# Ryan-Yanlong/DREAM-GNN

Hardware: AMD Instinct MI355X
Metric: GCMC+FGCN SpMM edges/sec and achieved HBM GB/s at 1/2/4/8 MI355X (higher is better)
Workload: dtype f32

## Files before the change

### dream_gnn_amd/csrc/dgmi_api.hip

```cpp
#include <hip/hip_runtime.h>
#include <limits.h>
#include <stdlib.h>
#include <string.h>

#include "dgmi.h"
#include "dgmi_bf16.h"
#include "dgmi_keep.h"
#include "dgmi_kernels.h"
#include "dgmi_tuning.h"

namespace {

inline hipStream_t as_stream(dgmi_stream_t s) { return static_cast<hipStream_t>(s); }

inline int from_hip(hipError_t e) { return e == hipSuccess ? DGMI_OK : DGMI_ERR_LAUNCH; }

long long env_ll(const char* name, long long dflt) {
  const char* e = getenv(name);
  return e != nullptr && e[0] != '\0' ? atoll(e) : dflt;
}

}

namespace dgmi {

Tuning& tuning() {
  static Tuning t = [] {
    Tuning v;
    v.sliced_rows = (int)env_ll("DGMI_SLICED_ROWS", 0);
    v.sliced_touch_lead = (int)env_ll("DGMI_SLICED_PF", -1);
    v.sliced_lpr = (int)env_ll("DGMI_SLICED_LPR", 0);
    v.sliced_no_off32 = getenv("DGMI_NO_OFF32") != nullptr ? 1 : 0;
    v.sliced_chunk_rows = env_ll("DGMI_SLICED_CHUNK_ROWS", 0);
    v.sliced_taper_rows = env_ll("DGMI_SLICED_TAPER_ROWS", 0);
    v.select_window_min = env_ll("DGMI_SELECT_WINDOW_MIN", 0);
    v.select_narrow_window = env_ll("DGMI_SELECT_NARROW_WINDOW", 0) != 0 ? 1 : 0;
    v.sort_plain_tiles = env_ll("DGMI_SORT_PLAIN_TILES", 0) != 0 ? 1 : 0;
    v.knn_screen_first = env_ll("DGMI_KNN_SCREEN_V1", 0) != 0 ? 1 : 0;
    v.knn_pool_chunks = env_ll("DGMI_KNN_POOL_CHUNKS", 0);
    return v;
  }();
  return t;
}

}

extern "C" {

DGMI_API int dgmi_set_tuning(const char* name, int64_t value) {
  if (name == nullptr) return DGMI_ERR_INVALID_ARG;
  dgmi::Tuning& t = dgmi::tuning();
  if (strcmp(name, "sliced_rows") == 0) t.sliced_rows = (int)value;
  else if (strcmp(name, "sliced_touch_lead") == 0) t.sliced_touch_lead = (int)value;
  else if (strcmp(name, "sliced_lpr") == 0) t.sliced_lpr = (int)value;
  else if (strcmp(name, "sliced_no_off32") == 0) t.sliced_no_off32 = value != 0;
  else if (strcmp(name, "sliced_chunk_rows") == 0) t.sliced_chunk_rows = value;
  else if (strcmp(name, "sliced_taper_rows") == 0) t.sliced_taper_rows = value;
  else if (strcmp(name, "select_window_min") == 0) t.select_window_min = value;
  else if (strcmp(name, "select_narrow_window") == 0) t.select_narrow_window = value != 0;
  else if (strcmp(name, "sort_plain_tiles") == 0) t.sort_plain_tiles = value != 0;
  else if (strcmp(name, "knn_screen_first") == 0) t.knn_screen_first = value != 0;
  else if (strcmp(name, "knn_pool_chunks") == 0) t.knn_pool_chunks = value;
  else return DGMI_ERR_INVALID_ARG;
  return DGMI_OK;
}

DGMI_API int dgmi_abi_version(void) { return DGMI_ABI_VERSION; }

DGMI_API const char* dgmi_status_string(int status) {
  switch (status) {
    case DGMI_OK: return "ok";
    case DGMI_ERR_INVALID_ARG: return "invalid argument (null pointer, negative size or ld < F)";
    case DGMI_ERR_TOO_LARGE: return "size does not fit the int32 id space";
    case DGMI_ERR_WORKSPACE: return "workspace missing or too small";
    case DGMI_ERR_LAUNCH: return "HIP launch failed";
    case DGMI_ERR_NO_DEVICE: return "no gfx950 device visible";
    default: return "unknown dgmi status";
  }
}

DGMI_API int dgmi_device_ok(void) {
  int n = 0;
  if (hipGetDeviceCount(&n) != hipSuccess || n <= 0) return 0;
  int dev = 0;
  if (hipGetDevice(&dev) != hipSuccess) return 0;
  hipDeviceProp_t prop;
  if (hipGetDeviceProperties(&prop, dev) != hipSuccess) return 0;
  return strncmp(prop.gcnArchName, "gfx950", 6) == 0 ? 1 : 0;
}

DGMI_API int dgmi_csr_from_coo_i32(const int32_t* row, const int32_t* col, int64_t E, int64_t n_rows,
                          int64_t n_cols, int32_t* indptr, int32_t* indices, int32_t* eid, void* workspace,
                          size_t* workspace_bytes, dgmi_stream_t stream) {
  if (E < 0 || n_rows < 0 || workspace_bytes == nullptr) return DGMI_ERR_INVALID_ARG;
  if (E > INT32_MAX || n_rows >= INT32_MAX || n_cols >= INT32_MAX) return DGMI_ERR_TOO_LARGE;
  if (workspace != nullptr) {
    if (indptr == nullptr) return DGMI_ERR_INVALID_ARG;
    if (E > 0 && (row == nullptr || col == nullptr || indices == nullptr || eid == nullptr))
      return DGMI_ERR_INVALID_ARG;
  }
  size_t need = 0;
  hipError_t err = dgmi::csr_from_coo_i32(row, col, E, n_rows, n_cols, indptr, indices, eid, nullptr,
                                          &need, as_stream(stream));
  if (err != hipSuccess) return DGMI_ERR_LAUNCH;
  if (workspace == nullptr) {
    *workspace_bytes = need;
    return DGMI_OK;
  }
  if (*workspace_bytes < need) return DGMI_ERR_WORKSPACE;
  return from_hip(dgmi::csr_from_coo_i32(row, col, E, n_rows, n_cols, indptr, indices, eid, workspace,
                                         workspace_bytes, as_stream(stream)));
}

static bool epilogue_ok(int32_t act, const float* out_mask, int64_t ld_mask, int64_t F) {
  return (act == 0 || act == 1) && (out_mask == nullptr || ld_mask >= F);
}

static bool keep_args_ok(const int32_t* eid, const uint32_t* keep, int32_t n_keep) {
  if (n_keep < 0 || n_keep > dgmi::kMaxKeepSegs) return false;
  return n_keep == 0 || (eid != nullptr && keep != nullptr);
}

DGMI_API int dgmi_spmm_csr_f32(const int32_t* indptr, const int32_t* indices, const float* vals,
                      const int32_t* eid, const uint32_t* keep, int32_t n_keep,
                      const float* X, int64_t ldx, const float* src_scale,
                      const float* dst_scale, float* Y, int64_t ldy, int64_t n_dst,
                      int64_t n_src, int64_t F, int32_t act, float act_slope, const float* out_mask,
                      int64_t ld_mask, float out_mask_scale, dgmi_stream_t stream) {
  if (n_dst < 0 || n_src < 0 || F < 0 || !keep_args_ok(eid, keep, n_keep) || !epilogue_ok(act, out_mask, ld_mask, F))
    return DGMI_ERR_INVALID_ARG;
  if (n_dst >= INT32_MAX || n_src >= INT32_MAX || F > INT32_MAX) return DGMI_ERR_TOO_LARGE;
  if (n_dst == 0 || F == 0) return DGMI_OK;
  if (indptr == nullptr || Y == nullptr) return DGMI_ERR_INVALID_ARG;
  if (ldx < F || ldy < F) return DGMI_ERR_INVALID_ARG;
  if (X == nullptr && n_src > 0) return DGMI_ERR_INVALID_ARG;
  if (static_cast<const void*>(X) == static_cast<const void*>(Y)) return DGMI_ERR_INVALID_ARG;
  dgmi::SpmmArgs a{indptr, indices, vals, X, ldx, src_scale, dst_scale, Y, ldy, n_dst, n_src, F,
                   nullptr, 0, 0, nullptr, 0, eid, keep, n_keep, {act, act_slope, out_mask, ld_mask, out_mask_scale}};
  return from_hip(dgmi::spmm_csr_f32(a, as_stream(stream)));
}

DGMI_API int32_t dgmi_spmm_default_chunk(int64_t n_rows, int64_t nnz) {
  (void)n_rows;
  int64_t c = (nnz / 4096 + 63) / 64 * 64;
  if (c < 64) c = 64;
  if (c > 512) c = 512;
  return (int32_t)c;
}

static bool chunk_ok(int32_t chunk) { return chunk >= 16 && chunk <= 65536; }

DGMI_API size_t dgmi_spmm_plan_bytes(int64_t n_rows, int64_t nnz, int32_t chunk) {
  if (n_rows < 0 || nnz < 0 || !chunk_ok(chunk)) return 0;
  return dgmi::plan_bytes(n_rows, nnz, chunk);
}

DGMI_API size_t dgmi_spmm_partials_bytes(int64_t nnz, int32_t chunk, int64_t F) {
  if (nnz < 0 || F < 0 || !chunk_ok(chunk)) return 0;
  const size_t ldp = (size_t)((F + 3) / 4 * 4);
  const size_t b = (size_t)dgmi::plan_slots_cap(nnz, chunk) * ldp * sizeof(float);
  return b < 16 ? 16 : b;
}

DGMI_API int dgmi_spmm_plan_build(const int32_t* indptr, int64_t n_rows, int64_t nnz, int32_t chunk,
                                  void* plan, size_t plan_bytes, void* workspace,
                                  size_t* workspace_bytes, dgmi_stream_t stream) {
  if (n_rows < 0 || nnz < 0 || !chunk_ok(chunk) || workspace_bytes == nullptr)
    return DGMI_ERR_INVALID_ARG;
  if (n_rows >= INT32_MAX || nnz > INT32_MAX) return DGMI_ERR_TOO_LARGE;
  size_t need = 0;
  if (dgmi::spmm_plan_build(indptr, n_rows, nnz, chunk, nullptr, nullptr, &need, as_stream(stream)) !=
      hipSuccess)
    return DGMI_ERR_LAUNCH;
  if (workspace == nullptr) {
    *workspace_bytes = need;
    return DGMI_OK;
  }
  if (plan == nullptr || (indptr == nullptr && n_rows > 0)) return DGMI_ERR_INVALID_ARG;
  if (*workspace_bytes < need || plan_bytes < dgmi::plan_bytes(n_rows, nnz, chunk))
    return DGMI_ERR_WORKSPACE;
  return from_hip(dgmi::spmm_plan_build(indptr, n_rows, nnz, chunk, static_cast<int32_t*>(plan),
                                        workspace, workspace_bytes, as_stream(stream)));
}

DGMI_API int dgmi_spmm_csr_planned_f32(const int32_t* indptr, const int32_t* indices,
                                       const float* vals, const int32_t* eid, const uint32_t* keep,
                                       int32_t n_keep, const float* X, int64_t ldx,
                                       const float* src_scale, const float* dst_scale, float* Y,
                                       int64_t ldy, int64_t n_dst, int64_t n_src, int64_t F,
                                       int64_t nnz, int32_t chunk, const void* plan, void* partials,
                                       size_t partials_bytes, int32_t act, float act_slope,
                                       const float* out_mask, int64_t ld_mask, float out_mask_scale,
                                       dgmi_stream_t stream) {
  if (n_dst < 0 || n_src < 0 || F < 0 || nnz < 0 || !chunk_ok(chunk) || !keep_args_ok(eid, keep, n_keep) ||
      !epilogue_ok(act, out_mask, ld_mask, F))
    return DGMI_ERR_INVALID_ARG;
  if (n_dst >= INT32_MAX || n_src >= INT32_MAX || F > INT32_MAX || nnz > INT32_MAX)
    return DGMI_ERR_TOO_LARGE;
  if (n_dst == 0 || F == 0) return DGMI_OK;
  if (indptr == nullptr || Y == nullptr || plan == nullptr || partials == nullptr)
    return DGMI_ERR_INVALID_ARG;
  if (ldx < F || ldy < F) return DGMI_ERR_INVALID_ARG;
  if (X == nullptr && n_src > 0) return DGMI_ERR_INVALID_ARG;
  if (static_cast<const void*>(X) == static_cast<const void*>(Y)) return DGMI_ERR_INVALID_ARG;
  if (partials_bytes < dgmi_spmm_partials_bytes(nnz, chunk, F)) return DGMI_ERR_WORKSPACE;
  dgmi::SpmmArgs a{indptr, indices, vals, X, ldx, src_scale, dst_scale, Y, ldy, n_dst, n_src, F,
                   static_cast<const int32_t*>(plan), nnz, chunk, static_cast<float*>(partials),
                   (F + 3) / 4 * 4, eid, keep, n_keep, {act, act_slope, out_mask, ld_mask, out_mask_scale}};
  return from_hip(dgmi::spmm_csr_f32(a, as_stream(stream)));
}

static int64_t slice_width_for(int64_t n_cols, int32_t n_slices) {
  const int64_t w = (n_cols + n_slices - 1) / n_slices;
  return w > 0 ? w : 1;
}

DGMI_API int dgmi_csr_sliced_from_coo_i32(const int32_t* row, const int32_t* col, int64_t E, int64_t n_rows,
                                          int64_t n_cols, int32_t n_slices, int32_t* segptr,
                                          int32_t* indices, int32_t* eid, void* workspace,
                                          size_t* workspace_bytes, dgmi_stream_t stream) {
  if (E < 0 || n_rows < 0 || n_cols < 0 || n_slices < 1 || n_slices > 64 || workspace_bytes == nullptr)
    return DGMI_ERR_INVALID_ARG;
  if (E > INT32_MAX || n_cols >= INT32_MAX || n_rows * (int64_t)n_slices >= INT32_MAX) return DGMI_ERR_TOO_LARGE;
  if (workspace != nullptr) {
    if (segptr == nullptr) return DGMI_ERR_INVALID_ARG;
    if (E > 0 && (row == nullptr || col == nullptr || indices == nullptr || eid == nullptr))
      return DGMI_ERR_INVALID_ARG;
  }
  const int64_t width = slice_width_for(n_cols, n_slices);
  size_t need = 0;
  if (dgmi::csr_sliced_from_coo_i32(row, col, E, n_rows, n_cols, n_slices, width, segptr, indices, eid, nullptr,
                                    &need, as_stream(stream)) != hipSuccess)
    return DGMI_ERR_LAUNCH;
  if (workspace == nullptr) {
    *workspace_bytes = need;
    return DGMI_OK;
  }
  if (*workspace_bytes < need) return DGMI_ERR_WORKSPACE;
  return from_hip(dgmi::csr_sliced_from_coo_i32(row, col, E, n_rows, n_cols, n_slices, width, segptr, indices,
                                                eid, workspace, workspace_bytes, as_stream(stream)));
}

DGMI_API int dgmi_csr_sliced_from_csr_i32(const int32_t* indptr, const int32_t* indices, const int32_t* eid, int64_t E,
                                          int64_t n_rows, int64_t n_cols, int32_t n_slices, int32_t* segptr,
                                          int32_t* s_indices, int32_t* s_eid, void* workspace, size_t* workspace_bytes,
                                          dgmi_stream_t stream) {
  if (E < 0 || n_rows < 0 || n_cols < 0 || n_slices < 1 || n_slices > 64 || workspace_bytes == nullptr)
    return DGMI_ERR_INVALID_ARG;
  if (E > INT32_MAX || n_cols >= INT32_MAX || n_rows * (int64_t)n_slices >= INT32_MAX) return DGMI_ERR_TOO_LARGE;
  if (workspace != nullptr) {
    if (segptr == nullptr) return DGMI_ERR_INVALID_ARG;
    if (E > 0 && (indptr == nullptr || indices == nullptr || eid == nullptr || s_indices == nullptr || s_eid == nullptr))
      return DGMI_ERR_INVALID_ARG;
  }
  const int64_t width = slice_width_for(n_cols, n_slices);
  size_t need = 0;
  if (dgmi::csr_sliced_from_csr_i32(indptr, indices, eid, E, n_rows, n_cols, n_slices, width, segptr, s_indices, s_eid,
                                    nullptr, &need, as_stream(stream)) != hipSuccess)
    return DGMI_ERR_LAUNCH;
  if (workspace == nullptr) {
    *workspace_bytes = need;
    return DGMI_OK;
  }
  if (*workspace_bytes < need) return DGMI_ERR_WORKSPACE;
  return from_hip(dgmi::csr_sliced_from_csr_i32(indptr, indices, eid, E, n_rows, n_cols, n_slices, width, segptr, s_indices,
                                                s_eid, workspace, workspace_bytes, as_stream(stream)));
}

static int64_t sliced_chunk_rows(int64_t n_dst, int32_t n_slices, int64_t F) {
  const int64_t row_bytes = (int64_t)n_slices * ((F + 3) / 4 * 4) * (int64_t)sizeof(float);
  int64_t rows = ((int64_t)4096 << 20) / (row_bytes > 0 ? row_bytes : 1);
  rows = rows / 1024 * 1024;
  if (rows < 1024) rows = 1024;
  if (dgmi::tuning().sliced_chunk_rows > 0) rows = dgmi::tuning().sliced_chunk_rows;
  return rows < n_dst ? rows : n_dst;
}

DGMI_API size_t dgmi_spmm_sliced_planes_bytes(int64_t n_dst, int32_t n_slices, int64_t F) {
  if (n_dst < 0 || n_slices < 1 || F < 0) return 0;
  const size_t b = (size_t)sliced_chunk_rows(n_dst, n_slices, F) * (size_t)n_slices *
                   (size_t)((F + 3) / 4 * 4) * sizeof(float);
  return b < 16 ? 16 : b;
}

static int spmm_sliced(const int32_t* segptr, const int32_t* indices, const float* vals, const int32_t* eid, const uint32_t* keep,
                       int32_t n_keep, const void* X, int x_bytes, int64_t ldx, const float* src_scale, const float* dst_scale,
                       float* Y, int64_t ldy, int64_t n_dst, int64_t n_src, int64_t F, int32_t n_slices, int32_t column_passes,
                       int32_t id_multiplicity, void* planes, size_t planes_bytes, int32_t act, float act_slope,
                       const float* out_mask, int64_t ld_mask, float out_mask_scale, dgmi_stream_t stream) {
  const int cols = 16 / x_bytes;
  if (n_dst < 0 || n_src < 0 || F < 0 || n_slices < 1 || n_slices > 64 || !keep_args_ok(eid, keep, n_keep) ||
      !epilogue_ok(act, out_mask, ld_mask, F) || column_passes < 0 || column_passes > 1 || id_multiplicity < 0 ||
      id_multiplicity > 1)
    return DGMI_ERR_INVALID_ARG;
  if (id_multiplicity == 1 && (vals != nullptr || n_src > (int64_t)dgmi::kMultIdMask + 1)) return DGMI_ERR_INVALID_ARG;
  if (out_mask != nullptr && (ld_mask % 4 != 0 || (reinterpret_cast<uintptr_t>(out_mask) & 15))) return DGMI_ERR_INVALID_ARG;
  if (n_dst >= INT32_MAX || n_src >= INT32_MAX || F > INT32_MAX) return DGMI_ERR_TOO_LARGE;
  if (n_dst == 0 || F == 0) return DGMI_OK;
  if (segptr == nullptr || Y == nullptr || planes == nullptr) return DGMI_ERR_INVALID_ARG;
  if (X == nullptr && n_src > 0) return DGMI_ERR_INVALID_ARG;
  if (ldx < F || ldy < F || F % cols != 0 || ldx % cols != 0 || ldy % 4 != 0) return DGMI_ERR_INVALID_ARG;
  if ((reinterpret_cast<uintptr_t>(X) & 15) || (reinterpret_cast<uintptr_t>(Y) & 15) ||
      (reinterpret_cast<uintptr_t>(planes) & 15))
    return DGMI_ERR_INVALID_ARG;
  if (X == static_cast<const void*>(Y)) return DGMI_ERR_INVALID_ARG;
  if (planes_bytes < dgmi_spmm_sliced_planes_bytes(n_dst, n_slices, F)) return DGMI_ERR_WORKSPACE;
  dgmi::SlicedArgs a{segptr, indices, vals, X, x_bytes, ldx, src_scale, dst_scale, Y, ldy, n_dst, n_src, F, n_slices,
                     static_cast<float*>(planes), F, sliced_chunk_rows(n_dst, n_slices, F), eid, keep, n_keep,
                     {act, act_slope, out_mask, ld_mask, out_mask_scale}, column_passes == 1, id_multiplicity == 1};
  return from_hip(x_bytes == 4 ? dgmi::spmm_sliced_f32(a, as_stream(stream)) : dgmi::spmm_sliced_bf16(a, as_stream(stream)));
}

DGMI_API int dgmi_spmm_sliced_f32(const int32_t* segptr, const int32_t* indices, const float* vals,
                                  const int32_t* eid, const uint32_t* keep, int32_t n_keep,
                                  const float* X, int64_t ldx, const float* src_scale,
                                  const float* dst_scale, float* Y, int64_t ldy, int64_t n_dst,
                                  int64_t n_src, int64_t F, int32_t n_slices, int32_t column_passes,
                                  int32_t id_multiplicity, void* planes,
                                  size_t planes_bytes, int32_t act, float act_slope, const float* out_mask,
                                  int64_t ld_mask, float out_mask_scale, dgmi_stream_t stream) {
  return spmm_sliced(segptr, indices, vals, eid, keep, n_keep, X, 4, ldx, src_scale, dst_scale, Y, ldy, n_dst, n_src, F,
                     n_slices, column_passes, id_multiplicity, planes, planes_bytes, act, act_slope, out_mask, ld_mask,
                     out_mask_scale, stream);
}

DGMI_API int dgmi_rows_to_bf16(const float* X, int64_t ldx, const float* scale, int64_t n, int64_t F, uint16_t* out, int64_t ldo,
                               dgmi_stream_t stream) {
  if (n < 0 || F < 0 || F % 8 != 0 || ldx < F || ldo < F || ldx % 4 != 0 || ldo % 8 != 0) return DGMI_ERR_INVALID_ARG;
  if (F > INT32_MAX) return DGMI_ERR_TOO_LARGE;
  if (n == 0 || F == 0) return DGMI_OK;
  if (X == nullptr || out == nullptr) return DGMI_ERR_INVALID_ARG;
  if ((reinterpret_cast<uintptr_t>(X) & 15) || (reinterpret_cast<uintptr_t>(out) & 15)) return DGMI_ERR_INVALID_ARG;
  if (static_cast<const void*>(X) == static_cast<const void*>(out)) return DGMI_ERR_INVALID_ARG;
  return from_hip(dgmi::rows_to_bf16(X, ldx, scale, n, F, out, ldo, as_stream(stream)));
}

DGMI_API int dgmi_spmm_sliced_bf16(const int32_t* segptr, const int32_t* indices, const float* vals, const int32_t* eid,
                                   const uint32_t* keep, int32_t n_keep, const uint16_t* X, int64_t ldx,
                                   const float* dst_scale, float* Y, int64_t ldy, int64_t n_dst, int64_t n_src, int64_t F,
                                   int32_t n_slices, int32_t column_passes, int32_t id_multiplicity, void* planes,
                                   size_t planes_bytes, int32_t act, float act_slope, const float* out_mask,
                                   int64_t ld_mask, float out_mask_scale, dgmi_stream_t stream) {
  return spmm_sliced(segptr, indices, vals, eid, keep, n_keep, X, 2, ldx, nullptr, dst_scale, Y, ldy, n_dst, n_src, F,
                     n_slices, column_passes, id_multiplicity, planes, planes_bytes, act, act_slope, out_mask, ld_mask,
                     out_mask_scale, stream);
}

DGMI_API int dgmi_gather_concat_f32(const int32_t* src, const int32_t* dst, int64_t E, const float* A,
                                    int64_t lda, int64_t Fa, const float* B, int64_t ldb, int64_t Fb,
                                    float* out, int64_t ldo, dgmi_stream_t stream) {
  if (E < 0 || Fa < 0 || Fb < 0) return DGMI_ERR_INVALID_ARG;
  if (E > INT32_MAX || Fa + Fb > INT32_MAX) return DGMI_ERR_TOO_LARGE;
  if (E == 0 || Fa + Fb == 0) return DGMI_OK;
  if (src == nullptr || dst == nullptr || out == nullptr) return DGMI_ERR_INVALID_ARG;
  if ((Fa > 0 && A == nullptr) || (Fb > 0 && B == nullptr)) return DGMI_ERR_INVALID_ARG;
  if (lda < Fa || ldb < Fb || ldo < Fa + Fb) return DGMI_ERR_INVALID_ARG;
  return from_hip(dgmi::gather_concat_f32(src, dst, E, A, lda, Fa, B, ldb, Fb, out, ldo, as_stream(stream)));
}

DGMI_API int dgmi_gather_add_f32(const int32_t* src, const int32_t* dst, int64_t E, const float* A,
// ... 177 lines not shown
```

### dream_gnn_amd/csrc/dgmi_sliced.hip

```cpp
#include <hip/hip_runtime.h>
#include <stdint.h>

#include "dgmi_sliced_common.h"

namespace dgmi {
namespace {

template <bool OFF32>
__device__ __forceinline__ float4 ld_row(const float* __restrict__ X, const float* __restrict__ Xc, int idx, int64_t ldx,
                                         uint32_t row_bytes, uint32_t col_bytes) {
  if (OFF32) return *reinterpret_cast<const float4*>(reinterpret_cast<const char*>(X) + ((uint32_t)idx * row_bytes + col_bytes));
  return ld4(Xc + (int64_t)idx * ldx);
}

template <int LPR, int VALS, bool HAS_SS, bool KEEP, bool OFF32>
__global__ __launch_bounds__(kWave* kWavesPerBlock) void spmm_sliced_vec4_kernel(
    const int32_t* __restrict__ segptr, const int32_t* __restrict__ indices,
    const float* __restrict__ vals, const float* __restrict__ X, int64_t ldx,
    const float* __restrict__ src_scale, float* __restrict__ planes, int64_t ldp, int64_t n_dst,
    int64_t row_begin, int64_t row_end, int F, int n_slices, const int32_t* __restrict__ eid,
    const KeepSeg* __restrict__ keep, int n_keep, int touch_lead, SlicedRuns runs, int touch_group) {
  constexpr int G = kWave / LPR;
  constexpr bool HAS_VALS = VALS == 1;
  constexpr bool MULT = VALS == 2;
  constexpr bool WEIGHTED = HAS_VALS || HAS_SS || MULT;
  constexpr bool W_LANE = HAS_VALS || HAS_SS;
  constexpr int kIdMask = MULT ? (int)kMultIdMask : 0x7fffffff;
  const int lane = threadIdx.x & (kWave - 1);
  const int wave = threadIdx.x >> 6;
  const int grp = lane / LPR, glane = lane % LPR, gbase = grp * LPR;
  const int slice = (int)(blockIdx.x % (unsigned)n_slices);
  int64_t block = blockIdx.x / (unsigned)n_slices;
  if (touch_group > 0 &&
      touch_ahead<HAS_VALS, KEEP>(segptr, indices, vals, eid, n_dst, row_begin, row_end, slice, runs, touch_lead, touch_group,
                                  lane, wave, block))
    return;
  const SlicedRun run = sliced_run(runs, block, wave * G + grp);
  const int nr = run.rows;
  if (nr == 0) return;
  const int64_t row0 = row_begin + run.first;
  int col = ((int)blockIdx.y * LPR + glane) * 4;
  const bool col_ok = col < F;
  if (!col_ok) col = 0;
  const float* Xc = X + col;
  const uint32_t row_bytes = (uint32_t)ldx * 4u, col_bytes = (uint32_t)col * 4u;
  const int32_t* sp = segptr + (int64_t)slice * n_dst + row0;
  float* prow = planes + ((int64_t)slice * (row_end - row_begin) + (row0 - row_begin)) * ldp + col;

  const KeepPre first = first_seg<KEEP>(keep, n_keep);
  const int my_b = sp[glane < nr ? glane : nr];
  const int e_begin = __shfl(my_b, gbase, kWave);
  const int e_end = __shfl(my_b, gbase + nr, kWave);
  int r = 0;
  int next_b = __shfl(my_b, gbase + 1, kWave);
  float4 acc = make_float4(0.f, 0.f, 0.f, 0.f);
  int nxt_idx = 0;
  float nxt_w = 0.f;
  int last_row = -1;
  if (e_begin < e_end) {
    const int q = e_begin + glane < e_end ? e_begin + glane : e_begin;
    nxt_idx = fetch_id<KEEP>(indices, eid, first, keep, n_keep, q);
    if (W_LANE) {
      nxt_w = HAS_VALS ? vals[q] : 1.f;
      if (HAS_SS) nxt_w *= src_scale[(KEEP || MULT) ? nxt_idx & kIdMask : nxt_idx];
    }
  }
  for (int base = e_begin; base < e_end; base += LPR) {
    const int n = min(LPR, e_end - base);
    const int my_idx = nxt_idx;
    const float my_w = nxt_w;
    if (base + LPR < e_end) {
      const int nb = base + LPR;
      const int q = nb + glane < e_end ? nb + glane : nb;
      nxt_idx = fetch_id<KEEP>(indices, eid, first, keep, n_keep, q);
      if (W_LANE) {
        nxt_w = HAS_VALS ? vals[q] : 1.f;
        if (HAS_SS) nxt_w *= src_scale[(KEEP || MULT) ? nxt_idx & kIdMask : nxt_idx];
      }
    }
    for (int j = 0; j < n; j += kUnroll) {
      float4 v[kUnroll];
      float w[kUnroll];
#pragma unroll
      for (int u = 0; u < kUnroll; ++u) {
        const int e = j + u;
        int idx = __shfl(my_idx, gbase + e, kWave);
        if (W_LANE) w[u] = __shfl(my_w, gbase + e, kWave);
        if (MULT) {
          const float m = (float)(((idx >> kMultShift) & kMultMax) + 1);
          w[u] = W_LANE ? w[u] * m : m;
        }
        const bool dropped = KEEP && idx < 0;
        if (KEEP) {
          idx = dropped && last_row >= 0 ? last_row : idx & kIdMask;
          last_row = idx;
        } else if (MULT) {
          idx &= kIdMask;
        }
        v[u] = ld_row<OFF32>(X, Xc, idx, ldx, row_bytes, col_bytes);
        if (dropped) v[u] = make_float4(0.f, 0.f, 0.f, 0.f);
      }
      if (base + j + kUnroll <= next_b) {
#pragma unroll
        for (int u = 0; u < kUnroll; ++u) {
          if (WEIGHTED) {
            acc.x = fmaf(w[u], v[u].x, acc.x);
            acc.y = fmaf(w[u], v[u].y, acc.y);
            acc.z = fmaf(w[u], v[u].z, acc.z);
            acc.w = fmaf(w[u], v[u].w, acc.w);
          } else {
            acc.x += v[u].x;
            acc.y += v[u].y;
            acc.z += v[u].z;
            acc.w += v[u].w;
          }
        }
        continue;
      }
#pragma unroll
      for (int u = 0; u < kUnroll; ++u) {
        const int p = base + j + u;
        if (p < e_end) {
          while (p >= next_b) {
            if (col_ok) store_plane_row(prow + (int64_t)r * ldp, acc);
            acc = make_float4(0.f, 0.f, 0.f, 0.f);
            ++r;
            next_b = __shfl(my_b, gbase + r + 1, kWave);
          }
          if (WEIGHTED) {
            acc.x = fmaf(w[u], v[u].x, acc.x);
            acc.y = fmaf(w[u], v[u].y, acc.y);
            acc.z = fmaf(w[u], v[u].z, acc.z);
            acc.w = fmaf(w[u], v[u].w, acc.w);
          } else {
            acc.x += v[u].x;
            acc.y += v[u].y;
            acc.z += v[u].z;
            acc.w += v[u].w;
          }
        }
      }
    }
  }
  for (; r < nr; ++r) {
    if (col_ok) store_plane_row(prow + (int64_t)r * ldp, acc);
    acc = make_float4(0.f, 0.f, 0.f, 0.f);
  }
}

template <bool HAS_DS, int S>
__global__ __launch_bounds__(256) void reduce_planes_kernel(const float* __restrict__ planes, int64_t ldp,
                                                            int64_t rows, int F4, int n_slices,
                                                            const float* __restrict__ dst_scale,
                                                            float* __restrict__ Y, int64_t ldy, Epilogue ep) {
  const int64_t total = rows * F4;
  const int64_t stride = (int64_t)gridDim.x * 256;
  const int64_t plane_stride = rows * ldp;
  const bool dense = (ldp == 4 * (int64_t)F4) && (ldy == ldp);
  for (int64_t t = (int64_t)blockIdx.x * 256 + threadIdx.x; t < total; t += stride) {
    int64_t row, poff, yoff;
    if (dense) {
      row = t / F4;
      poff = yoff = 4 * t;
    } else {
      row = t / F4;
      const int c = (int)(t - row * F4) * 4;
      poff = row * ldp + c;
      yoff = row * ldy + c;
    }
    const float* p = planes + poff;
    float4 acc;
    if (S > 0) {
      float4 v[S > 0 ? S : 1];
#pragma unroll
      for (int s = 0; s < S; ++s) {
        const v4f t = __builtin_nontemporal_load(reinterpret_cast<const v4f*>(p + s * plane_stride));
        v[s] = make_float4(t.x, t.y, t.z, t.w);
      }
      acc = v[0];
#pragma unroll
      for (int s = 1; s < S; ++s) {
        acc.x += v[s].x;
        acc.y += v[s].y;
        acc.z += v[s].z;
        acc.w += v[s].w;
      }
    } else {
      acc = *reinterpret_cast<const float4*>(p);
      for (int s = 1; s < n_slices; ++s) {
        const float4 v = *reinterpret_cast<const float4*>(p + s * plane_stride);
        acc.x += v.x;
        acc.y += v.y;
        acc.z += v.z;
        acc.w += v.w;
      }
    }
    if (HAS_DS) {
      const float d = dst_scale[row];
      acc.x *= d;
      acc.y *= d;
      acc.z *= d;
      acc.w *= d;
    }
    *reinterpret_cast<float4*>(Y + yoff) = epilogue4(ep, acc, row, (int)(yoff - row * ldy));
  }
}

hipError_t reduce_planes(const float* planes, int64_t ldp, int64_t rows, int64_t F, int64_t n_slices, const float* ds, float* y,
                         int64_t ldy, const Epilogue& ep, hipStream_t s) {
  const int F4 = (int)(F / 4);
  int64_t blocks = (rows * F4 + 255) / 256;
  if (blocks > 8192) blocks = 8192;
#define DGMI_REDUCE(D, S)                                                                                        \
  hipLaunchKernelGGL((reduce_planes_kernel<D, S>), dim3((unsigned)blocks), dim3(256), 0, s, planes, ldp, rows, F4, \
                     (int)n_slices, ds, y, ldy, ep)
  if (n_slices == 8) {
    if (ds) DGMI_REDUCE(true, 8); else DGMI_REDUCE(false, 8);
  } else {
    if (ds) DGMI_REDUCE(true, 0); else DGMI_REDUCE(false, 0);
  }
#undef DGMI_REDUCE
  return hipGetLastError();
}

template <int LPR>
hipError_t launch_sliced(const SlicedArgs& a, int64_t row_begin, int64_t row_end, hipStream_t s) {
  const SlicedGeometry g = sliced_geometry(row_begin, row_end, a.F, a.n_src, a.ldx, a.n_slices, LPR, a.x_bytes);
  dim3 block(kWave * kWavesPerBlock);
  const int key = (a.vals ? 4 : (a.id_mult ? 8 : 0)) | (a.src_scale ? 2 : 0) | (a.n_keep > 0 ? 1 : 0);
#define DGMI_LAUNCH_O(V, S, K, O)                                                                                      \
  hipLaunchKernelGGL((spmm_sliced_vec4_kernel<LPR, V, S, K, O>), g.grid, block, 0, s, a.segptr, a.indices, a.vals,      \
                     static_cast<const float*>(a.X), a.ldx, a.src_scale, a.planes, a.ldp, a.n_dst, row_begin, row_end, \
                     (int)a.F, (int)a.n_slices, a.eid, static_cast<const KeepSeg*>(a.keep), a.n_keep, g.touch_lead, g.runs, \
                     g.touch_group)
#define DGMI_LAUNCH(V, S, K)                                              \
  do {                                                                    \
    if (g.off32) DGMI_LAUNCH_O(V, S, K, true); else DGMI_LAUNCH_O(V, S, K, false); \
  } while (0)
  switch (key) {
    case 0: DGMI_LAUNCH(0, false, false); break;
    case 1: DGMI_LAUNCH(0, false, true); break;
    case 2: DGMI_LAUNCH(0, true, false); break;
    case 3: DGMI_LAUNCH(0, true, true); break;
    case 4: DGMI_LAUNCH(1, false, false); break;
    case 5: DGMI_LAUNCH(1, false, true); break;
    case 6: DGMI_LAUNCH(1, true, false); break;
    case 7: DGMI_LAUNCH(1, true, true); break;
    case 8: DGMI_LAUNCH(2, false, false); break;
    case 9: DGMI_LAUNCH(2, false, true); break;
    case 10: DGMI_LAUNCH(2, true, false); break;
    default: DGMI_LAUNCH(2, true, true); break;
  }
#undef DGMI_LAUNCH
#undef DGMI_LAUNCH_O
  return hipGetLastError();
}

hipError_t launch_gather_f32(const SlicedArgs& a, int lpr, int64_t r0, int64_t r1, hipStream_t s) {
  switch (lpr) {
    case 8: return launch_sliced<8>(a, r0, r1, s);
    case 16: return launch_sliced<16>(a, r0, r1, s);
    case 32: return launch_sliced<32>(a, r0, r1, s);
    default: return launch_sliced<64>(a, r0, r1, s);
  }
}

}

hipError_t spmm_sliced_chunks(const SlicedArgs& a, SlicedGather gather, hipStream_t s) {
  if (a.n_dst == 0 || a.F == 0) return hipSuccess;
  const int64_t chunk = a.chunk_rows > 0 ? a.chunk_rows : a.n_dst;
  for (int64_t r0 = 0; r0 < a.n_dst; r0 += chunk) {
    const int64_t r1 = r0 + chunk < a.n_dst ? r0 + chunk : a.n_dst;
    const int lpr = sliced_lpr(a.F, a.n_src, a.n_slices, a.n_dst, a.full_width, a.n_keep, a.x_bytes, tuning().sliced_lpr);
    hipError_t err = gather(a, lpr, r0, r1, s);
    if (err != hipSuccess) return err;
    Epilogue ep = a.ep;
    if (ep.mask != nullptr) ep.mask += r0 * ep.ldm;
    err = reduce_planes(a.planes, a.ldp, r1 - r0, a.F, a.n_slices, a.dst_scale ? a.dst_scale + r0 : nullptr, a.Y + r0 * a.ldy,
                        a.ldy, ep, s);
    if (err != hipSuccess) return err;
  }
  return hipSuccess;
}

hipError_t spmm_sliced_f32(const SlicedArgs& a, hipStream_t s) {
  if (a.x_bytes != 4) return hipErrorInvalidValue;
  return spmm_sliced_chunks(a, launch_gather_f32, s);
}

}
```

### dream_gnn_amd/csrc/dgmi_sliced_common.h

```cpp
#pragma once
#include <hip/hip_runtime.h>
#include <stdint.h>

#include "dgmi_kernels.h"
#include "dgmi_segment.h"
#include "dgmi_tuning.h"

namespace dgmi {

typedef hipError_t (*SlicedGather)(const SlicedArgs& a, int lpr, int64_t row_begin, int64_t row_end, hipStream_t s);

hipError_t spmm_sliced_chunks(const SlicedArgs& a, SlicedGather gather, hipStream_t s);

namespace {

constexpr int64_t kColumnPassMinRows = 32768;
constexpr int kRowsPerGroup = 8;
constexpr int64_t kTaperRows = 8192;
constexpr int kTouchLead = 24;
constexpr int kTouchGroup = 8;

typedef float v4f __attribute__((ext_vector_type(4)));

__device__ __forceinline__ void store_plane_row(float* p, const float4& v) {
  v4f t = {v.x, v.y, v.z, v.w};
  __builtin_nontemporal_store(t, reinterpret_cast<v4f*>(p));
}

struct SlicedRuns {
  int64_t end[3];
  int64_t blocks[3];
  int run[3];
  int groups;
};

struct SlicedRun {
  int64_t first;
  int rows;
};

__host__ __device__ inline SlicedRuns sliced_runs(int64_t n_rows, int R, int G, int64_t taper) {
  SlicedRuns t;
  taper = taper < 0 ? 0 : (taper < n_rows ? taper : n_rows);
  t.groups = kWavesPerBlock * G;
  t.run[0] = R;
  t.run[1] = (R + 1) / 2;
  t.run[2] = (R + 3) / 4;
  t.end[0] = n_rows - taper;
  t.end[1] = n_rows - taper / 2;
  t.end[2] = n_rows;
  int64_t blocks = 0, begin = 0;
  for (int s = 0; s < 3; ++s) {
    const int64_t per_block = (int64_t)t.groups * t.run[s];
    blocks += (t.end[s] - begin + per_block - 1) / per_block;
    t.blocks[s] = blocks;
    begin = t.end[s];
  }
  return t;
}

__host__ __device__ inline SlicedRun sliced_run(const SlicedRuns& t, int64_t block, int slot) {
  const int s = block < t.blocks[0] ? 0 : (block < t.blocks[1] ? 1 : 2);
  const int64_t begin = s > 0 ? t.end[s - 1] : 0, block0 = s > 0 ? t.blocks[s - 1] : 0;
  const int64_t first = begin + ((block - block0) * t.groups + slot) * t.run[s];
  if (block >= t.blocks[2] || first >= t.end[s]) return SlicedRun{t.end[2], 0};
  const int64_t left = t.end[s] - first;
  return SlicedRun{first, (int)(left < t.run[s] ? left : t.run[s])};
}

template <bool HAS_VALS, bool KEEP>
__device__ __forceinline__ bool touch_ahead(const int32_t* __restrict__ segptr, const int32_t* __restrict__ indices,
                                            const float* __restrict__ vals, const int32_t* __restrict__ eid, int64_t n_dst,
                                            int64_t row_begin, int64_t row_end, int slice, const SlicedRuns& runs,
                                            int touch_lead, int touch_group, int lane, int wave, int64_t& block) {
  const int64_t t = block / (touch_group + 1);
  if (block % (touch_group + 1) == 0) {
    __shared__ int range[2];
    const int32_t* sp_s = segptr + (int64_t)slice * n_dst;
    const int64_t ahead = t * touch_group + touch_lead;
    const int64_t r_first = row_begin + sliced_run(runs, ahead, 0).first;
    if (r_first >= row_end) return true;
    const int64_t r_last = row_begin + sliced_run(runs, ahead + touch_group, 0).first;
    int keepalive = 0;
    if (wave == 0) {
      const int64_t rp = lane == 0 ? r_first : (lane == 1 ? r_last : r_first + (int64_t)(lane - 1) * 32);
      if (rp <= r_last) {
        const int v = sp_s[rp];
        if (lane < 2) range[lane] = v;
        keepalive = v;
      }
    }
    __syncthreads();
    const int e0 = range[0], e1 = range[1];
    for (int64_t p = (int64_t)e0 + (int64_t)threadIdx.x * 32; p < e1; p += (int64_t)blockDim.x * 32) {
      keepalive ^= indices[p];
      if (HAS_VALS) keepalive ^= __float_as_int(vals[p]);
      if (KEEP) keepalive ^= eid[p];
    }
    asm volatile("" ::"v"(keepalive));
    return true;
  }
  block -= t + 1;
  return false;
}

inline int rows_per_group(int lpr) {
  (void)lpr;
  return kRowsPerGroup;
}

struct SlicedGeometry {
  int R;
  SlicedRuns runs;
  int64_t workers;
  int64_t touchers;
  dim3 grid;
  int touch_lead, touch_group;
  bool off32;
};

inline SlicedGeometry sliced_geometry(int64_t row_begin, int64_t row_end, int64_t F, int64_t n_src, int64_t ldx,
                                      int64_t n_slices, int lpr, int elem_bytes) {
  SlicedGeometry g;
  const int G = kWave / lpr, cols = 16 / elem_bytes;
  const Tuning& tune = tuning();
  const int rows_req = tune.sliced_rows > 0 ? tune.sliced_rows : rows_per_group(lpr);
  g.R = rows_req < 1 ? 1 : (rows_req < lpr ? rows_req : lpr - 1);
  const int64_t quarter = (row_end - row_begin) / 4;
  const int64_t taper = tune.sliced_taper_rows < 0 ? 0
                        : (tune.sliced_taper_rows > 0 ? tune.sliced_taper_rows : (kTaperRows < quarter ? kTaperRows : quarter));
  g.runs = sliced_runs(row_end - row_begin, g.R, G, taper);
  g.workers = g.runs.blocks[2];
  g.off32 = !tune.sliced_no_off32 && (n_src * ldx + F) * elem_bytes < ((int64_t)1 << 32);
  g.touch_lead = tune.sliced_touch_lead >= 0 ? tune.sliced_touch_lead : kTouchLead;
  g.touch_group = g.touch_lead > 0 ? kTouchGroup : 0;
  g.touchers = g.touch_group > 0 ? (g.workers + g.touch_group - 1) / g.touch_group : 0;
  g.grid = dim3((unsigned)((g.workers + g.touchers) * n_slices), (unsigned)((F + cols * lpr - 1) / (cols * lpr)));
  return g;
}

inline int sliced_lpr(int64_t F, int64_t n_src, int64_t n_slices, int64_t n_dst, bool full_width, int n_keep, int elem_bytes,
                      int forced) {
  const int cols = 16 / elem_bytes, widest = 256 / cols;
  int lpr = pick_lpr(F, cols, widest);
  if (lpr >= 32 && !full_width && n_keep == 0 && n_dst >= kColumnPassMinRows) {
    const int64_t width = 16 * (int64_t)lpr < elem_bytes * F ? 16 * (int64_t)lpr : elem_bytes * F;
    const int64_t slice_bytes = (n_src + n_slices - 1) / n_slices * width;
    if (slice_bytes > (4 << 20)) lpr /= 2;
  }
  if (forced == 8 || forced == 16 || forced == 32 || (forced == 64 && widest == 64)) lpr = forced;
  return lpr;
}

}
}
```

### dream_gnn_amd/csrc/dgmi_tuning.h

```cpp
#pragma once
#include <stdint.h>

namespace dgmi {

struct Tuning {
  int sliced_rows = 0;
  int sliced_touch_lead = -1;
  int sliced_lpr = 0;
  int sliced_no_off32 = 0;
  int64_t sliced_chunk_rows = 0;
  int64_t sliced_taper_rows = 0;
  int64_t select_window_min = 0;
  int select_narrow_window = 0;
  int sort_plain_tiles = 0;
  int knn_screen_first = 0;
  int64_t knn_pool_chunks = 0;
};

Tuning& tuning();

}
```

Baseline: 33.48 billion.

## Add persistent owned-row SpMM kernel accumulating slices in LDS

Adds a persistent kernel with one workgroup per CU. Each workgroup owns a block of destination rows and keeps their partial sums in LDS across the eight source slices, so per-slice planes are no longer written to HBM and then reduced in a second pass. A dedicated wave prefetches segment pointers and indices ahead of the workers. Workgroups are loosely phase-synchronised through global arrival counters with a timed spin fallback. The path runs by default only for a narrow class (8 slices, unweighted, 16–32 MB feature table, two row rounds). It adds cross-workgroup spinning and LDS capacity limits as risks.

Measured after the change: 34.32 billion, median of 6. +2.5%, better.

```diff
diff --git a/dream_gnn_amd/csrc/dgmi_api.hip b/dream_gnn_amd/csrc/dgmi_api.hip
--- a/dream_gnn_amd/csrc/dgmi_api.hip
+++ b/dream_gnn_amd/csrc/dgmi_api.hip
@@ -33,6 +33,12 @@
     v.sliced_no_off32 = getenv("DGMI_NO_OFF32") != nullptr ? 1 : 0;
     v.sliced_chunk_rows = env_ll("DGMI_SLICED_CHUNK_ROWS", 0);
     v.sliced_taper_rows = env_ll("DGMI_SLICED_TAPER_ROWS", 0);
+    v.sliced_owned = (int)env_ll("DGMI_SLICED_OWNED", -1);
+    v.sliced_owned_grid = (int)env_ll("DGMI_SLICED_OWNED_GRID", 0);
+    v.sliced_owned_rows = (int)env_ll("DGMI_SLICED_OWNED_ROWS", 0);
+    v.sliced_owned_lds_rows = env_ll("DGMI_SLICED_OWNED_LDS_ROWS", 0);
+    v.sliced_owned_lag = (int)env_ll("DGMI_SLICED_OWNED_LAG", -2);
+    v.sliced_owned_spin_ticks = env_ll("DGMI_SLICED_OWNED_SPIN_TICKS", 0);
     v.select_window_min = env_ll("DGMI_SELECT_WINDOW_MIN", 0);
     v.select_narrow_window = env_ll("DGMI_SELECT_NARROW_WINDOW", 0) != 0 ? 1 : 0;
     v.sort_plain_tiles = env_ll("DGMI_SORT_PLAIN_TILES", 0) != 0 ? 1 : 0;
@@ -56,6 +62,12 @@
   else if (strcmp(name, "sliced_no_off32") == 0) t.sliced_no_off32 = value != 0;
   else if (strcmp(name, "sliced_chunk_rows") == 0) t.sliced_chunk_rows = value;
   else if (strcmp(name, "sliced_taper_rows") == 0) t.sliced_taper_rows = value;
+  else if (strcmp(name, "sliced_owned") == 0) t.sliced_owned = (int)value;
+  else if (strcmp(name, "sliced_owned_grid") == 0) t.sliced_owned_grid = (int)value;
+  else if (strcmp(name, "sliced_owned_rows") == 0) t.sliced_owned_rows = (int)value;
+  else if (strcmp(name, "sliced_owned_lds_rows") == 0) t.sliced_owned_lds_rows = value;
+  else if (strcmp(name, "sliced_owned_lag") == 0) t.sliced_owned_lag = (int)value;
+  else if (strcmp(name, "sliced_owned_spin_ticks") == 0) t.sliced_owned_spin_ticks = value;
   else if (strcmp(name, "select_window_min") == 0) t.select_window_min = value;
   else if (strcmp(name, "select_narrow_window") == 0) t.select_narrow_window = value != 0;
   else if (strcmp(name, "sort_plain_tiles") == 0) t.sort_plain_tiles = value != 0;
diff --git a/dream_gnn_amd/csrc/dgmi_owned.hip b/dream_gnn_amd/csrc/dgmi_owned.hip
--- /dev/null
+++ b/dream_gnn_amd/csrc/dgmi_owned.hip
@@ -0,0 +1,333 @@
+#include <hip/hip_runtime.h>
+#include <stdint.h>
+
+#include "dgmi_owned_common.h"
+#include "dgmi_sliced_common.h"
+
+namespace dgmi {
+namespace {
+
+constexpr int kOwnedTouchChunk = 4;
+constexpr int kOwnedTouchLead = 8;
+constexpr int64_t kOwnedSpinTicks = 3000;
+constexpr int64_t kOwnedMinRows = 32768;
+constexpr int kOwnedLag = -1;
+
+struct OwnedWork {
+  int phase, task, slice, col_round;
+  int64_t row0;
+  int lds_row, rows;
+};
+
+__device__ __forceinline__ OwnedWork owned_decode(const OwnedPlan& pl, int64_t wg, int T, int k, int grp) {
+  OwnedWork w;
+  w.phase = k / T;
+  w.task = k - w.phase * T;
+  const OwnedPhase ph = owned_phase(pl, w.phase);
+  w.slice = ph.slice;
+  w.col_round = ph.col_round;
+  const OwnedTask t = owned_task(pl, wg, ph.row_round, w.task, grp);
+  w.row0 = t.row0;
+  w.lds_row = t.lds_row;
+  w.rows = t.rows;
+  return w;
+}
+
+template <int LPR, int VALS, bool OFF32>
+__global__ __launch_bounds__(kWave* kOwnedWaves) void spmm_owned_kernel(
+    const int32_t* __restrict__ segptr, const int32_t* __restrict__ indices, const float* __restrict__ X, int64_t ldx,
+    const float* __restrict__ dst_scale, float* __restrict__ Y, int64_t ldy, int64_t n_dst, int F, OwnedPlan pl,
+    unsigned* __restrict__ arrive, int lag, int64_t spin_ticks, Epilogue ep) {
+  constexpr bool MULT = VALS == 2;
+  constexpr int kIdMask = MULT ? (int)kMultIdMask : 0x7fffffff;
+  extern __shared__ float4 lds_rows[];
+  const int lane = threadIdx.x & (kWave - 1);
+  const int wave = threadIdx.x >> 6;
+  const int grp = lane / LPR, glane = lane % LPR, gbase = grp * LPR;
+  const int64_t wg = blockIdx.x;
+  const int T = owned_wg_tasks(pl, wg);
+  if (T == 0) return;
+  int* done = reinterpret_cast<int*>(lds_rows + (size_t)pl.round_rows * LPR);
+  int* phase_cnt = done + pl.tasks;
+  int* counter = phase_cnt + pl.phases;
+  int* open = counter + 1;
+  for (int i = threadIdx.x; i < pl.tasks + pl.phases + 2; i += blockDim.x) done[i] = 0;
+  __syncthreads();
+  const int total = pl.phases * T;
+  const int label = (int)(blockIdx.x & 7u);
+  const unsigned n_label = (unsigned)((pl.active - label + 7) >> 3);
+  unsigned* my_arrive = arrive + (size_t)label * pl.phases;
+
+  if (wave == kOwnedWaves - 1) {
+    const int chunks_per_phase = (T + kOwnedTouchChunk - 1) / kOwnedTouchChunk, chunks = pl.phases * chunks_per_phase;
+    const int last_gate = lag >= 0 ? pl.phases - 1 : 0;
+    int keepalive = 0, touched = 0, opened = 0;
+    bool waiting = false;
+    uint64_t wait_start = 0;
+    while (touched < chunks || opened < last_gate) {
+      bool idle = true;
+      const int next = __hip_atomic_load(counter, __ATOMIC_RELAXED, __HIP_MEMORY_SCOPE_WORKGROUP);
+      if (touched < chunks) {
+        const int P = touched / chunks_per_phase, t0 = (touched - P * chunks_per_phase) * kOwnedTouchChunk;
+        if (P * T + t0 <= next + kOwnedTouchLead) {
+          ++touched;
+          idle = false;
+          const OwnedPhase ph = owned_phase(pl, P);
+          const int64_t in_round = owned_round_rows(pl, wg, ph.row_round);
+          const int64_t lds_first = (int64_t)t0 * pl.G * pl.R;
+          int64_t lds_last = lds_first + (int64_t)kOwnedTouchChunk * pl.G * pl.R;
+          if (lds_last > in_round) lds_last = in_round;
+          if (lds_first < lds_last) {
+            const int32_t* sp_s = segptr + (int64_t)ph.slice * n_dst;
+            const int64_t r_first = owned_task(pl, wg, ph.row_round, t0, 0).row0, r_last = r_first + (lds_last - lds_first);
+            const int64_t rp = lane == 0 ? r_first : (lane == 1 ? r_last : r_first + (int64_t)(lane - 1) * 32);
+            int v = 0;
+            if (rp <= r_last) v = sp_s[rp];
+            keepalive ^= v;
+            const int e0 = __builtin_amdgcn_readlane(v, 0), e1 = __builtin_amdgcn_readlane(v, 1);
+            for (int64_t p = (int64_t)e0 + (int64_t)lane * 32; p < e1; p += (int64_t)kWave * 32) keepalive ^= indices[p];
+            asm volatile("" ::"v"(keepalive));
+          }
+        }
+      }
+      if (opened < last_gate) {
+        const int P = opened + 1, need = P - 1 - lag;
+        bool ok = need < 0 || __hip_atomic_load(&my_arrive[need], __ATOMIC_RELAXED, __HIP_MEMORY_SCOPE_AGENT) >= n_label;
+        if (!ok && next >= P * T) {
+          const uint64_t now = __builtin_amdgcn_s_memrealtime();
+          if (!waiting) {
+            waiting = true;
+            wait_start = now;
+          } else if (now - wait_start >= (uint64_t)spin_ticks) {
+            ok = true;
+          }
+        }
+        if (ok) {
+          opened = P;
+          waiting = false;
+          idle = false;
+          __hip_atomic_store(open, P, __ATOMIC_RELAXED, __HIP_MEMORY_SCOPE_WORKGROUP);
+        }
+      }
+      if (idle) __builtin_amdgcn_s_sleep(2);
+    }
+    return;
+  }
+
+  auto grab = [&]() {
+    int k = 0;
+    if (lane == 0) k = __hip_atomic_fetch_add(counter, 1, __ATOMIC_RELAXED, __HIP_MEMORY_SCOPE_WORKGROUP);
+    return __builtin_amdgcn_readfirstlane(k);
+  };
+  auto boundaries = [&](int k) {
+    if (k >= total) return 0;
+    const OwnedWork w = owned_decode(pl, wg, T, k, grp);
+    if (w.rows == 0) return 0;
+    return segptr[(int64_t)w.slice * n_dst + w.row0 + (glane < w.rows ? glane : w.rows)];
+  };
+  auto first_ids = [&](int my_b, int rows) {
+    const int e_begin = __shfl(my_b, gbase, kWave), e_end = __shfl(my_b, gbase + rows, kWave);
+    if (rows == 0 || e_begin >= e_end) return 0;
+    return indices[e_begin + glane < e_end ? e_begin + glane : e_begin];
+  };
+
+  const uint32_t row_bytes = (uint32_t)ldx * 4u;
+  int k = grab();
+  int my_b = boundaries(k);
+  int nxt_idx = k < total ? first_ids(my_b, owned_decode(pl, wg, T, k, grp).rows) : 0;
+  while (k < total) {
+    const OwnedWork w = owned_decode(pl, wg, T, k, grp);
+    const int k_next = grab();
+    const int next_b = boundaries(k_next);
+    if (lag >= 0)
+      while (__hip_atomic_load(open, __ATOMIC_RELAXED, __HIP_MEMORY_SCOPE_WORKGROUP) < w.phase) __builtin_amdgcn_s_sleep(1);
+    while (__hip_atomic_load(&done[w.task], __ATOMIC_ACQUIRE, __HIP_MEMORY_SCOPE_WORKGROUP) < w.phase) __builtin_amdgcn_s_sleep(1);
+
+    const int nr = w.rows;
+    int col = (w.col_round * LPR + glane) * 4;
+    const bool col_ok = col < F;
+    if (!col_ok) col = 0;
+    const float* Xc = X + col;
+    const uint32_t col_bytes = (uint32_t)col * 4u;
+    float4* slot = lds_rows + (size_t)w.lds_row * LPR + glane;
+    auto commit = [&](int r, const float4& acc) {
+      if (w.slice == 0) {
+        slot[r * LPR] = acc;
+        return;
+      }
+      float4 t = slot[r * LPR];
+      t.x += acc.x;
+      t.y += acc.y;
+      t.z += acc.z;
+      t.w += acc.w;
+      if (w.slice < kOwnedSlices - 1) {
+        slot[r * LPR] = t;
+        return;
+      }
+      if (col_ok) {
+        const int64_t row = w.row0 + r;
+        if (dst_scale != nullptr) {
+          const float d = dst_scale[row];
+          t.x *= d;
+          t.y *= d;
+          t.z *= d;
+          t.w *= d;
+        }
+        *reinterpret_cast<float4*>(Y + row * ldy + col) = epilogue4(ep, t, row, col);
+      }
+    };
+
+    if (nr > 0) {
+      const int e_begin = __shfl(my_b, gbase, kWave);
+      const int e_end = __shfl(my_b, gbase + nr, kWave);
+      int r = 0;
+      int row_end = __shfl(my_b, gbase + 1, kWave);
+      float4 acc = make_float4(0.f, 0.f, 0.f, 0.f);
+      for (int base = e_begin; base < e_end; base += LPR) {
+        const int n = min(LPR, e_end - base);
+        const int my_idx = nxt_idx;
+        if (base + LPR < e_end) {
+          const int nb = base + LPR;
+          nxt_idx = indices[nb + glane < e_end ? nb + glane : nb];
+        }
+        for (int j = 0; j < n; j += kUnroll) {
+          float4 v[kUnroll];
+          float m[kUnroll];
+#pragma unroll
+          for (int u = 0; u < kUnroll; ++u) {
+            int idx = __shfl(my_idx, gbase + j + u, kWave);
+            if (MULT) {
+              m[u] = (float)(((idx >> kMultShift) & kMultMax) + 1);
+              idx &= kIdMask;
+            }
+            v[u] = ld_row<OFF32>(X, Xc, idx, ldx, row_bytes, col_bytes);
+          }
+          if (base + j + kUnroll <= row_end) {
+#pragma unroll
+            for (int u = 0; u < kUnroll; ++u) {
+              if (MULT) {
+                acc.x = fmaf(m[u], v[u].x, acc.x);
+                acc.y = fmaf(m[u], v[u].y, acc.y);
+                acc.z = fmaf(m[u], v[u].z, acc.z);
+                acc.w = fmaf(m[u], v[u].w, acc.w);
+              } else {
+                acc.x += v[u].x;
+                acc.y += v[u].y;
+                acc.z += v[u].z;
+                acc.w += v[u].w;
+              }
+            }
+            continue;
+          }
+#pragma unroll
+          for (int u = 0; u < kUnroll; ++u) {
+            const int p = base + j + u;
+            if (p < e_end) {
+              while (p >= row_end) {
+                commit(r, acc);
+                acc = make_float4(0.f, 0.f, 0.f, 0.f);
+                ++r;
+                row_end = __shfl(my_b, gbase + r + 1, kWave);
+              }
+              if (MULT) {
+                acc.x = fmaf(m[u], v[u].x, acc.x);
+                acc.y = fmaf(m[u], v[u].y, acc.y);
+                acc.z = fmaf(m[u], v[u].z, acc.z);
+                acc.w = fmaf(m[u], v[u].w, acc.w);
+              } else {
+                acc.x += v[u].x;
+                acc.y += v[u].y;
+                acc.z += v[u].z;
+                acc.w += v[u].w;
+              }
+            }
+          }
+        }
+      }
+      for (; r < nr; ++r) {
+        commit(r, acc);
+        acc = make_float4(0.f, 0.f, 0.f, 0.f);
+      }
+    }
+    nxt_idx = k_next < total ? first_ids(next_b, owned_decode(pl, wg, T, k_next, grp).rows) : 0;
+    __builtin_amdgcn_wave_barrier();
+    if (lane == 0) {
+      __hip_atomic_store(&done[w.task], w.phase + 1, __ATOMIC_RELEASE, __HIP_MEMORY_SCOPE_WORKGROUP);
+      const int finished = __hip_atomic_fetch_add(&phase_cnt[w.phase], 1, __ATOMIC_RELAXED, __HIP_MEMORY_SCOPE_WORKGROUP);
+      if (finished == T - 1) __hip_atomic_fetch_add(&my_arrive[w.phase], 1u, __ATOMIC_RELAXED, __HIP_MEMORY_SCOPE_AGENT);
+    }
+    k = k_next;
+    my_b = next_b;
+  }
+}
+
+int device_cus() {
+  static const int cus = [] {
+    int dev = 0, n = 0;
+    if (hipGetDevice(&dev) != hipSuccess || hipDeviceGetAttribute(&n, hipDeviceAttributeMultiprocessorCount, dev) != hipSuccess)
+      return 0;
+    return n;
+  }();
+  return cus;
+}
+
+bool owned_class_selected(const OwnedPlan& pl, bool id_mult, int64_t table_bytes) {
+  return pl.col_rounds == 1 && pl.row_rounds == 2 && !id_mult && table_bytes >= ((int64_t)16 << 20) && table_bytes <= ((int64_t)32 << 20);
+}
+
+template <int LPR>
+hipError_t launch_owned(const SlicedArgs& a, const OwnedPlan& pl, int64_t grid, bool off32, int lag, int64_t spin_ticks,
+                        hipStream_t s) {
+  unsigned* arrive = reinterpret_cast<unsigned*>(a.planes);
+  hipError_t err = hipMemsetAsync(arrive, 0, sizeof(unsigned) * 8 * (size_t)pl.phases, s);
+  if (err != hipSuccess) return err;
+#define DGMI_OWNED(V, O)                                                                                                  \
+  do {                                                                                                                    \
+    auto kern = spmm_owned_kernel<LPR, V, O>;                                                                             \
+    static const hipError_t attr = hipFuncSetAttribute(reinterpret_cast<const void*>(kern),                               \
+                                                       hipFuncAttributeMaxDynamicSharedMemorySize, 160 << 10);            \
+    if (attr != hipSuccess) return attr;                                                                                  \
+    hipLaunchKernelGGL(kern, dim3((unsigned)grid), dim3(kWave* kOwnedWaves), pl.lds_bytes, s, a.segptr, a.indices,        \
+                       static_cast<const float*>(a.X), a.ldx, a.dst_scale, a.Y, a.ldy, a.n_dst, (int)a.F, pl, arrive, lag, \
+                       spin_ticks, a.ep);                                                                                 \
+  } while (0)
+  if (a.id_mult) {
+    if (off32) DGMI_OWNED(2, true); else DGMI_OWNED(2, false);
+  } else {
+    if (off32) DGMI_OWNED(0, true); else DGMI_OWNED(0, false);
+  }
+#undef DGMI_OWNED
+  return hipGetLastError();
+}
+
+}
+
+hipError_t spmm_owned_try(const SlicedArgs& a, hipStream_t s, bool* taken) {
+  *taken = false;
+  const Tuning& tune = tuning();
+  if (tune.sliced_owned == 0) return hipSuccess;
+  if (a.x_bytes != 4 || a.vals != nullptr || a.src_scale != nullptr || a.n_keep != 0 || a.n_slices != kOwnedSlices ||
+      tune.sliced_chunk_rows > 0 || a.chunk_rows < a.n_dst || a.n_dst == 0 || a.F == 0)
+    return hipSuccess;
+  const int64_t grid = tune.sliced_owned_grid > 0 ? tune.sliced_owned_grid : device_cus();
+  if (grid < 1) return hipSuccess;
+  const int lpr = sliced_lpr(a.F, a.n_src, a.n_slices, a.n_dst, a.full_width, a.n_keep, a.x_bytes, tune.sliced_lpr);
+  const OwnedPlan pl = owned_plan(a.n_dst, a.F, lpr, grid, tune.sliced_owned_rows, tune.sliced_owned_lds_rows);
+  if (!pl.ok || pl.lds_bytes > (size_t)(160 << 10)) return hipSuccess;
+  if (sizeof(unsigned) * 8 * (size_t)pl.phases > sizeof(float) * (size_t)a.n_slices * (size_t)a.n_dst * (size_t)a.ldp) return hipSuccess;
+  if (tune.sliced_owned != 1 &&
+      (a.n_dst < kOwnedMinRows || !owned_class_selected(pl, a.id_mult, a.n_src * a.ldx * (int64_t)sizeof(float))))
+    return hipSuccess;
+  const bool off32 = !tune.sliced_no_off32 && (a.n_src * a.ldx + a.F) * 4 < ((int64_t)1 << 32);
+  const int64_t spin = tune.sliced_owned_spin_ticks > 0 ? tune.sliced_owned_spin_ticks : kOwnedSpinTicks;
+  const int lag = tune.sliced_owned_lag >= -1 ? tune.sliced_owned_lag : kOwnedLag;
+  *taken = true;
+  switch (lpr) {
+    case 8: return launch_owned<8>(a, pl, grid, off32, lag, spin, s);
+    case 16: return launch_owned<16>(a, pl, grid, off32, lag, spin, s);
+    case 32: return launch_owned<32>(a, pl, grid, off32, lag, spin, s);
+    default: return launch_owned<64>(a, pl, grid, off32, lag, spin, s);
+  }
+}
+
+}
diff --git a/dream_gnn_amd/csrc/dgmi_owned_common.h b/dream_gnn_amd/csrc/dgmi_owned_common.h
--- /dev/null
+++ b/dream_gnn_amd/csrc/dgmi_owned_common.h
@@ -0,0 +1,97 @@
+#pragma once
+#include <hip/hip_runtime.h>
+#include <stddef.h>
+#include <stdint.h>
+
+namespace dgmi {
+
+constexpr int kOwnedSlices = 8;
+constexpr int kOwnedWaves = 16;
+constexpr int kOwnedWorkers = kOwnedWaves - 1;
+constexpr int64_t kOwnedLdsRowBytes = 144 << 10;
+constexpr int kOwnedMaxPhases = 128;
+constexpr int kOwnedPhaseTasks = 24;
+constexpr int kOwnedMaxRows = 8;
+
+struct OwnedPlan {
+  bool ok;
+  int lpr, G, R;
+  int col_rounds, row_rounds, phases;
+  int64_t wg_rows;
+  int64_t active;
+  int round_rows;
+  int tasks;
+  int64_t n_dst;
+  size_t lds_bytes;
+};
+
+struct OwnedPhase {
+  int col_round, row_round, slice;
+};
+
+struct OwnedTask {
+  int64_t row0;
+  int lds_row;
+  int rows;
+};
+
+__host__ __device__ inline OwnedPlan owned_plan(int64_t n_dst, int64_t F, int lpr, int64_t grid, int R_req, int64_t lds_rows_cap) {
+  OwnedPlan p{};
+  p.ok = false;
+  p.n_dst = n_dst;
+  if (n_dst < 1 || F < 1 || grid < 1 || (lpr != 8 && lpr != 16 && lpr != 32 && lpr != 64)) return p;
+  p.lpr = lpr;
+  p.G = 64 / lpr;
+  p.col_rounds = (int)((F + 4 * lpr - 1) / (4 * lpr));
+  p.wg_rows = (n_dst + grid - 1) / grid;
+  p.active = (n_dst + p.wg_rows - 1) / p.wg_rows;
+  int64_t fit = kOwnedLdsRowBytes / (16 * lpr);
+  if (lds_rows_cap > 0 && lds_rows_cap < fit) fit = lds_rows_cap;
+  const int64_t rounds = (p.wg_rows + fit - 1) / fit;
+  if (rounds * p.col_rounds * kOwnedSlices > kOwnedMaxPhases) return p;
+  p.row_rounds = (int)rounds;
+  p.round_rows = (int)((p.wg_rows + rounds - 1) / rounds);
+  p.phases = p.col_rounds * p.row_rounds * kOwnedSlices;
+  int R = R_req;
+  if (R <= 0) {
+    R = (p.round_rows + kOwnedPhaseTasks * p.G / 2) / (kOwnedPhaseTasks * p.G);
+    if (R > kOwnedMaxRows) R = kOwnedMaxRows;
+  }
+  if (R > lpr - 1) R = lpr - 1;
+  if (R < 1) R = 1;
+  p.R = R;
+  p.tasks = (p.round_rows + p.G * R - 1) / (p.G * R);
+  p.lds_bytes = (size_t)p.round_rows * 16 * lpr + sizeof(int) * ((size_t)p.tasks + p.phases + 2);
+  p.ok = true;
+  return p;
+}
+
+__host__ __device__ inline int64_t owned_wg_rows(const OwnedPlan& p, int64_t wg) {
+  const int64_t left = p.n_dst - wg * p.wg_rows;
+  return left < 0 ? 0 : (left < p.wg_rows ? left : p.wg_rows);
+}
+
+__host__ __device__ inline int64_t owned_round_rows(const OwnedPlan& p, int64_t wg, int row_round) {
+  const int64_t left = owned_wg_rows(p, wg) - (int64_t)row_round * p.round_rows;
+  return left < 0 ? 0 : (left < p.round_rows ? left : p.round_rows);
+}
+
+__host__ __device__ inline int owned_wg_tasks(const OwnedPlan& p, int64_t wg) {
+  int64_t rows = owned_wg_rows(p, wg);
+  if (rows > p.round_rows) rows = p.round_rows;
+  return (int)((rows + p.G * p.R - 1) / (p.G * p.R));
+}
+
+__host__ __device__ inline OwnedPhase owned_phase(const OwnedPlan& p, int phase) {
+  const int cq = phase / kOwnedSlices;
+  return OwnedPhase{cq / p.row_rounds, cq % p.row_rounds, phase % kOwnedSlices};
+}
+
+__host__ __device__ inline OwnedTask owned_task(const OwnedPlan& p, int64_t wg, int row_round, int task, int group) {
+  const int64_t lds_row = ((int64_t)task * p.G + group) * p.R;
+  int64_t rows = owned_round_rows(p, wg, row_round) - lds_row;
+  rows = rows < 0 ? 0 : (rows < p.R ? rows : p.R);
+  return OwnedTask{wg * p.wg_rows + (int64_t)row_round * p.round_rows + lds_row, (int)lds_row, (int)rows};
+}
+
+}
diff --git a/dream_gnn_amd/csrc/dgmi_sliced.hip b/dream_gnn_amd/csrc/dgmi_sliced.hip
--- a/dream_gnn_amd/csrc/dgmi_sliced.hip
+++ b/dream_gnn_amd/csrc/dgmi_sliced.hip
@@ -5,13 +5,6 @@
 
 namespace dgmi {
 namespace {
-
-template <bool OFF32>
-__device__ __forceinline__ float4 ld_row(const float* __restrict__ X, const float* __restrict__ Xc, int idx, int64_t ldx,
-                                         uint32_t row_bytes, uint32_t col_bytes) {
-  if (OFF32) return *reinterpret_cast<const float4*>(reinterpret_cast<const char*>(X) + ((uint32_t)idx * row_bytes + col_bytes));
-  return ld4(Xc + (int64_t)idx * ldx);
-}
 
 template <int LPR, int VALS, bool HAS_SS, bool KEEP, bool OFF32>
 __global__ __launch_bounds__(kWave* kWavesPerBlock) void spmm_sliced_vec4_kernel(
@@ -286,6 +279,9 @@
 
 hipError_t spmm_sliced_f32(const SlicedArgs& a, hipStream_t s) {
   if (a.x_bytes != 4) return hipErrorInvalidValue;
+  bool owned = false;
+  const hipError_t err = spmm_owned_try(a, s, &owned);
+  if (err != hipSuccess || owned) return err;
   return spmm_sliced_chunks(a, launch_gather_f32, s);
 }
 
diff --git a/dream_gnn_amd/csrc/dgmi_sliced_common.h b/dream_gnn_amd/csrc/dgmi_sliced_common.h
--- a/dream_gnn_amd/csrc/dgmi_sliced_common.h
+++ b/dream_gnn_amd/csrc/dgmi_sliced_common.h
@@ -12,6 +12,8 @@
 
 hipError_t spmm_sliced_chunks(const SlicedArgs& a, SlicedGather gather, hipStream_t s);
 
+hipError_t spmm_owned_try(const SlicedArgs& a, hipStream_t s, bool* taken);
+
 namespace {
 
 constexpr int64_t kColumnPassMinRows = 32768;
@@ -25,6 +27,13 @@
 __device__ __forceinline__ void store_plane_row(float* p, const float4& v) {
   v4f t = {v.x, v.y, v.z, v.w};
   __builtin_nontemporal_store(t, reinterpret_cast<v4f*>(p));
+}
+
+template <bool OFF32>
+__device__ __forceinline__ float4 ld_row(const float* __restrict__ X, const float* __restrict__ Xc, int idx, int64_t ldx,
+                                         uint32_t row_bytes, uint32_t col_bytes) {
+  if (OFF32) return *reinterpret_cast<const float4*>(reinterpret_cast<const char*>(X) + ((uint32_t)idx * row_bytes + col_bytes));
+  return ld4(Xc + (int64_t)idx * ldx);
 }
 
 struct SlicedRuns {
diff --git a/dream_gnn_amd/csrc/dgmi_tuning.h b/dream_gnn_amd/csrc/dgmi_tuning.h
--- a/dream_gnn_amd/csrc/dgmi_tuning.h
+++ b/dream_gnn_amd/csrc/dgmi_tuning.h
@@ -10,6 +10,12 @@
   int sliced_no_off32 = 0;
   int64_t sliced_chunk_rows = 0;
   int64_t sliced_taper_rows = 0;
+  int sliced_owned = -1;
+  int sliced_owned_grid = 0;
+  int sliced_owned_rows = 0;
+  int64_t sliced_owned_lds_rows = 0;
+  int sliced_owned_lag = -2;
+  int64_t sliced_owned_spin_ticks = 0;
   int64_t select_window_min = 0;
   int select_narrow_window = 0;
   int sort_plain_tiles = 0;
```
